# emtiyaz/vmp-for-svae

Measured on AMD Instinct MI355X. Metric: vmp_step_datapoints_per_sec, higher is better.
Workload: dtype f32

## Files before the change

vmp-for-svae_amd/csrc/vmp_mix.hip:

```cpp
#include "vmp_common.h"
#include "vmp_linalg.h"
#include <stdlib.h>
#include <type_traits>

using namespace vmp;

namespace {

constexpr int TR = 64;
constexpr int LS = 68;
constexpr int MAX_NW = 8;
constexpr int MAX_NW1 = 8;
constexpr int max_nw(int KT) { return KT == 1 ? MAX_NW1 : MAX_NW; }
constexpr int MAX_BLOCKS = 1024;

struct PassArgs {
    const float* x;
    const float* r_in;
    const float* u_in;
    const uint8_t* mask;
    const float* pivot;
    const float* pack;
    float* r_out;
    float* u_out;
    float* logr_out;
    double* partials;
    long long N;
    long long rpw;
    long long rpw_b;
    int K;
    int vec_ok;
    int par_reduce;
#ifdef VMP_DEBUG_TS
    long long* dbg_t;
#endif
};
#ifdef VMP_DEBUG_TS
#define PASS_TS(i) do { if (a.dbg_t && (blockIdx.x == 0 || blockIdx.x == 100) && (threadIdx.x & 63) == 0) { a.dbg_t[(blockIdx.x ? 64 : 0) + (threadIdx.x >> 6) * 8 + (i)] = clock64(); \
    if ((i) == 0 && threadIdx.x == 0) a.dbg_t[(blockIdx.x ? 64 : 0) + 7] = wall_clock64();           \
    if ((i) == 5 && threadIdx.x == 64) a.dbg_t[(blockIdx.x ? 64 : 0) + 8 + 7] = wall_clock64(); } } while (0)
#else
#define PASS_TS(i) do { } while (0)
#endif

#define VMP_DPP2(OP, CTRL)                                                   \
    "v_" OP "_f32_dpp %0, %0, %0 " CTRL " row_mask:0xf bank_mask:0xf\n\t"  \
    "v_" OP "_f32_dpp %1, %1, %1 " CTRL " row_mask:0xf bank_mask:0xf\n\t"  \
    "s_nop 0\n\t"
#define VMP_DPP2_FIRST(OP, CTRL)                                             \
    "v_" OP "_f32_dpp %0, %2, %2 " CTRL " row_mask:0xf bank_mask:0xf\n\t"  \
    "v_" OP "_f32_dpp %1, %3, %3 " CTRL " row_mask:0xf bank_mask:0xf\n\t"  \
    "s_nop 0\n\t"
__device__ __forceinline__ v2f row16_max2(v2f v) {
    float a, b;
    asm("s_nop 1\n\t" VMP_DPP2_FIRST("max", "row_ror:8") VMP_DPP2("max", "row_ror:4") VMP_DPP2("max", "row_ror:2")
        VMP_DPP2("max", "row_ror:1")
        : "=&v"(a), "=&v"(b) : "v"(v.x), "v"(v.y));
    return v2f{a, b};
}
__device__ __forceinline__ v2f row16_sum2(v2f v) {
    float a, b;
    asm("s_nop 1\n\t" VMP_DPP2_FIRST("add", "row_ror:8") VMP_DPP2("add", "row_ror:4") VMP_DPP2("add", "row_ror:2")
        VMP_DPP2("add", "row_ror:1")
        : "=&v"(a), "=&v"(b) : "v"(v.x), "v"(v.y));
    return v2f{a, b};
}

#define VMP_DPP4(OP, CTRL)                                                   \
    "v_" OP "_f32_dpp %0, %0, %0 " CTRL " row_mask:0xf bank_mask:0xf\n\t"  \
    "v_" OP "_f32_dpp %1, %1, %1 " CTRL " row_mask:0xf bank_mask:0xf\n\t"  \
    "v_" OP "_f32_dpp %2, %2, %2 " CTRL " row_mask:0xf bank_mask:0xf\n\t"  \
    "v_" OP "_f32_dpp %3, %3, %3 " CTRL " row_mask:0xf bank_mask:0xf\n\t"
#define VMP_DPP4_FIRST(OP, CTRL)                                             \
    "v_" OP "_f32_dpp %0, %4, %4 " CTRL " row_mask:0xf bank_mask:0xf\n\t"  \
    "v_" OP "_f32_dpp %1, %5, %5 " CTRL " row_mask:0xf bank_mask:0xf\n\t"  \
    "v_" OP "_f32_dpp %2, %6, %6 " CTRL " row_mask:0xf bank_mask:0xf\n\t"  \
    "v_" OP "_f32_dpp %3, %7, %7 " CTRL " row_mask:0xf bank_mask:0xf\n\t"
[[maybe_unused]] __device__ __forceinline__ void row16_max4(v2f v0, v2f v1, v2f& o0, v2f& o1) {
    float a, b, c, d;
    asm("s_nop 1\n\t" VMP_DPP4_FIRST("max", "row_ror:8") VMP_DPP4("max", "row_ror:4") VMP_DPP4("max", "row_ror:2")
        VMP_DPP4("max", "row_ror:1")
        : "=&v"(a), "=&v"(b), "=&v"(c), "=&v"(d) : "v"(v0.x), "v"(v0.y), "v"(v1.x), "v"(v1.y));
    o0 = v2f{a, b};
    o1 = v2f{c, d};
}
[[maybe_unused]] __device__ __forceinline__ void row16_sum4(v2f v0, v2f v1, v2f& o0, v2f& o1) {
    float a, b, c, d;
    asm("s_nop 1\n\t" VMP_DPP4_FIRST("add", "row_ror:8") VMP_DPP4("add", "row_ror:4") VMP_DPP4("add", "row_ror:2")
        VMP_DPP4("add", "row_ror:1")
        : "=&v"(a), "=&v"(b), "=&v"(c), "=&v"(d) : "v"(v0.x), "v"(v0.y), "v"(v1.x), "v"(v1.y));
    o0 = v2f{a, b};
    o1 = v2f{c, d};
}

#define VMP_RS4(OP, TAIL)                                                                   \
    "s_nop 1\n\t"                                                                           \
    "v_" OP "_f32_dpp %0, %3, %3 row_ror:8 row_mask:0xf bank_mask:0x3\n\t"                \
    "v_" OP "_f32_dpp %0, %5, %5 row_ror:8 row_mask:0xf bank_mask:0xc\n\t"                \
    "v_" OP "_f32_dpp %1, %4, %4 row_ror:8 row_mask:0xf bank_mask:0x3\n\t"                \
    "v_" OP "_f32_dpp %1, %6, %6 row_ror:8 row_mask:0xf bank_mask:0xc\n\t"                \
    "v_" OP "_f32_dpp %2, %0, %0 row_ror:12 row_mask:0xf bank_mask:0x5\n\t"               \
    "s_nop 0\n\t"                                                                           \
    "v_" OP "_f32_dpp %2, %1, %1 row_ror:4 row_mask:0xf bank_mask:0xa\n\t"                \
    "s_nop 1\n\t"                                                                           \
    "v_" OP "_f32_dpp %2, %2, %2 quad_perm:[2,3,0,1] row_mask:0xf bank_mask:0xf\n\t"      \
    "s_nop 1\n\t"                                                                           \
    "v_" OP "_f32_dpp %2, %2, %2 quad_perm:[1,0,3,2] row_mask:0xf bank_mask:0xf\n\t" TAIL
__device__ __forceinline__ float row16_rs4_max(v2f v0, v2f v1) {
    float a0, a1, b;
    asm(VMP_RS4("max", "s_nop 1\n\t") : "=&v"(a0), "=&v"(a1), "=&v"(b) : "v"(v0.x), "v"(v0.y), "v"(v1.x), "v"(v1.y));
    return b;
}
__device__ __forceinline__ float row16_rs4_sum(v2f v0, v2f v1) {
    float a0, a1, b;
    asm(VMP_RS4("add", "") : "=&v"(a0), "=&v"(a1), "=&v"(b) : "v"(v0.x), "v"(v0.y), "v"(v1.x), "v"(v1.y));
    return b;
}
template <int V>
__device__ __forceinline__ float row16_bcast_bank(float s) {
    return __uint_as_float(__builtin_amdgcn_update_dpp(0u, __float_as_uint(s), 0x150 + 4 * V, 0xf, 0xf, true));
}

#ifndef VMP_PASS_PIPE
#define VMP_PASS_PIPE 4
#endif

constexpr int MOM_TERMS = 3;
#ifndef VMP_MOM_FLUSH
#define VMP_MOM_FLUSH 2
#endif

template <int D, int KT, int FLAV>
__device__ __forceinline__ void pass_epilogue(const PassArgs& a, float* smem, const double (&dacc)[KT][Geo<D>::FT][4],
                                              const double (&dn)[KT][4], int lane, int wave, int nw) {
    using G = Geo<D>;
    constexpr int FT = G::FT;
    constexpr bool SMM = (FLAV == VMP_SMM);
    const int K = a.K;
    {
        __syncthreads();
        PASS_TS(3);
        double* sc = reinterpret_cast<double*>(smem);
        constexpr int SLAB = KT * (FT + 1) * 4 * WAVE;
        if (a.par_reduce) {
            double* mine = sc + wave * SLAB;
#pragma unroll
            for (int kt = 0; kt < KT; ++kt)
#pragma unroll
                for (int c = 0; c < 4; ++c) {
#pragma unroll
                    for (int ft = 0; ft < FT; ++ft) mine[((kt * (FT + 1) + ft) * 4 + c) * WAVE + lane] = dacc[kt][ft][c];
                    mine[((kt * (FT + 1) + FT) * 4 + c) * WAVE + lane] = SMM ? dn[kt][c] : dacc[kt][0][c];
                }
            __syncthreads();
            constexpr int EPT = 2, NWB = max_nw(KT);
            for (int e0 = threadIdx.x; e0 < SLAB; e0 += EPT * blockDim.x) {
                double vals[EPT][NWB];
#pragma unroll
                for (int q = 0; q < EPT; ++q) {
                    const int e = e0 + q * blockDim.x;
#pragma unroll
                    for (int w = 0; w < NWB; ++w) vals[q][w] = (e < SLAB && w < nw) ? sc[w * SLAB + e] : 0.0;
                }
#pragma unroll
                for (int q = 0; q < EPT; ++q) {
                    const int e = e0 + q * blockDim.x;
                    double t2 = vals[q][0];
#pragma unroll
                    for (int w = 1; w < NWB; ++w) t2 += vals[q][w];
                    if (e < SLAB) sc[e] = t2;
                }
            }
            __syncthreads();
        } else {
            for (int w = 0; w < nw; ++w) {
                if (wave == w) {
#pragma unroll
                    for (int kt = 0; kt < KT; ++kt)
#pragma unroll
                        for (int c = 0; c < 4; ++c) {
#pragma unroll
                            for (int ft = 0; ft < FT; ++ft) {
                                const int idx = ((kt * (FT + 1) + ft) * 4 + c) * WAVE + lane;
                                sc[idx] = (w == 0 ? 0.0 : sc[idx]) + dacc[kt][ft][c];
                            }
                            const int idn = ((kt * (FT + 1) + FT) * 4 + c) * WAVE + lane;
                            sc[idn] = (w == 0 ? 0.0 : sc[idn]) + (SMM ? dn[kt][c] : dacc[kt][0][c]);
                        }
                }
                __syncthreads();
            }
        }
        PASS_TS(4);
        constexpr int PX = G::PF + 1;
        double* out = a.partials;
        for (int e = threadIdx.x; e < KT * (FT + 1) * 4 * WAVE; e += blockDim.x) {
            const int l = e & 63, c = (e >> 6) & 3, tf = (e >> 8) % (FT + 1), kt = (e >> 8) / (FT + 1);
            const int k = kt * 16 + (l >> 4) * 4 + c;
            if (k >= K) continue;
            double* row = out + ((long long)k * MAX_BLOCKS + blockIdx.x) * PX;
            if (tf < FT) {
                const int f = tf * 16 + (l & 15);
                if (f < G::F) row[f] = sc[e];
            } else if ((l & 15) == 0) {
                row[G::F] = sc[e];
            }
        }
        if (wave == 0) {
// ... 338 lines not shown
                        av[t] = __builtin_bit_cast(bf16x8, u32x4{As[kt][t][0], As[kt][t][1], As[kt][t][2], As[kt][t][3]});
                        if constexpr (SMM) rv[t] = __builtin_bit_cast(bf16x8, u32x4{Rs[kt][t][0], Rs[kt][t][1], Rs[kt][t][2], Rs[kt][t][3]});
                    }
#pragma unroll
                    for (int ta = 0; ta < MOM_TERMS; ++ta) {
#pragma unroll
                        for (int tb = 0; tb + ta < MOM_TERMS; ++tb) {
#pragma unroll
                            for (int ft = 0; ft < FT; ++ft) {
                                if (ta + tb == 0) acc[kt][ft] = __builtin_amdgcn_mfma_f32_16x16x32_bf16(av[ta], b[ft][tb], acc[kt][ft], 0, 0, 0);
                                else acs[kt][ft] = __builtin_amdgcn_mfma_f32_16x16x32_bf16(av[ta], b[ft][tb], acs[kt][ft], 0, 0, 0);
                            }
                        }
                        if constexpr (SMM) {
                            if (ta == 0) nacc[kt] = __builtin_amdgcn_mfma_f32_16x16x32_bf16(rv[ta], b[0][0], nacc[kt], 0, 0, 0);
                            else nacs[kt] = __builtin_amdgcn_mfma_f32_16x16x32_bf16(rv[ta], b[0][0], nacs[kt], 0, 0, 0);
                        }
                    }
                }
            }
        }

        if constexpr (STATS) {
            if (((row0 - lo) / TR) % VMP_MOM_FLUSH == VMP_MOM_FLUSH - 1 || row0 + TR >= hi) {
#pragma unroll
                for (int kt = 0; kt < KT; ++kt) {
#pragma unroll
                    for (int c = 0; c < 4; ++c) {
                        if constexpr (SMM) dn[kt][c] += (double)nacc[kt][c] + (double)nacs[kt][c];
#pragma unroll
                        for (int ft = 0; ft < FT; ++ft) dacc[kt][ft][c] += (double)acc[kt][ft][c] + (double)acs[kt][ft][c];
                    }
                    nacc[kt] = f32x4{0.f, 0.f, 0.f, 0.f};
                    nacs[kt] = f32x4{0.f, 0.f, 0.f, 0.f};
#pragma unroll
                    for (int ft = 0; ft < FT; ++ft) { acc[kt][ft] = f32x4{0.f, 0.f, 0.f, 0.f}; acs[kt][ft] = f32x4{0.f, 0.f, 0.f, 0.f}; }
                }
            }
        }
        __builtin_amdgcn_wave_barrier();
    }

    PASS_TS(2);
    if constexpr (STATS) pass_epilogue<D, KT, FLAV>(a, smem, dacc, dn, lane, wave, nw);
}


constexpr int AIS = 36;

struct FinArgs {
    const double* partials;
    const double* stats_in;
    int nblk, K, flavour, src, do_post;
    const float *alpha0, *beta0, *m0, *C0, *v0, *kappa;
    const float* pivot;
    float *alpha, *beta, *m, *C, *v, *xbar, *S, *pi, *pack;
    double* pack64;
    double* stats_out;
    double* peer[VMP_EXCH_MAX_RANKS];
    int nranks, rank;
    unsigned long long iter;
    int* status;
#ifdef VMP_DEBUG_TS
    long long* dbg_t;
#endif
};

#ifdef VMP_DEBUG_TS
#define FIN_TS(i) do { if (a.dbg_t && blockIdx.x == 0 && tid == 0) { a.dbg_t[i] = clock64(); if ((i) == 0) a.dbg_t[6] = wall_clock64(); if ((i) == 5) a.dbg_t[7] = wall_clock64(); } } while (0)
#else
#define FIN_TS(i) do { } while (0)
#endif
#ifdef VMP_DEBUG_TS
#define FIN_TSX(i, t) do { if (a.dbg_t && blockIdx.x == 0 && tid == (t)) a.dbg_t[i] = clock64(); } while (0)
#else
#define FIN_TSX(i, t) do { } while (0)
#endif

template <int D>
__device__ void finalize_block(const FinArgs& a, const int k, const int tid, const int nthreads);

template <int D> constexpr int xdl_wave_floats() { return Geo<D>::XROWS * LS + TR * AIS; }

template <int D, int FLAV, bool STATS, int MT = 3>
__device__ __forceinline__ void pass_xdl_body(const PassArgs& a) {
    using G = Geo<D>;
    constexpr int FT = G::FT, KT = 1;
    constexpr bool SMM = (FLAV == VMP_SMM);
    constexpr int DP = (D + 1) / 2;
    extern __shared__ __attribute__((aligned(16))) float smem[];
    const int lane = threadIdx.x & 63, wave = threadIdx.x >> 6, nw = blockDim.x >> 6;
    const int K = a.K;
    PASS_TS(0);
    float* xl = smem + wave * xdl_wave_floats<D>();
    unsigned* ai = reinterpret_cast<unsigned*>(xl + G::XROWS * LS);
    constexpr int ONE = D, ZERO = D + 1;
    const int ppos = (lane & ~15) + 4 * (lane & 3) + ((lane >> 2) & 3);

    const bool vec = a.vec_ok != 0;
    long long lo, hi;
    if (a.rpw_b == a.rpw) {
        lo = ((long long)blockIdx.x * nw + wave) * a.rpw;
        hi = lo + a.rpw;
    } else {
        const int hw = nw >> 1;
        const long long base = (long long)blockIdx.x * hw * (a.rpw + a.rpw_b);
        lo = wave < hw ? base + wave * a.rpw : base + hw * a.rpw + (wave - hw) * a.rpw_b;
        hi = lo + (wave < hw ? a.rpw : a.rpw_b);
    }
    if (hi > a.N) hi = a.N;
    float xr[D];
    {
        const long long n = lo + lane;
#pragma unroll
        for (int j = 0; j < D; ++j) xr[j] = 0.f;
        if (n < hi) load_row<D>(a.x + n * D, xr, vec);
    }
    const int i16 = lane & 15, kk = lane >> 4;
    float pv[D];
    {
        const float* __restrict__ pp = a.pivot ? a.pivot : a.x;
        const bool hasp = a.pivot != nullptr;
#pragma unroll
        for (int j = 0; j < D; ++j) { const float v = pp[j]; pv[j] = hasp ? v : 0.f; }
#pragma unroll
        for (int j = 0; j < D; ++j) pv[j] = __builtin_bit_cast(float, __builtin_amdgcn_readfirstlane(__builtin_bit_cast(int, pv[j])));
    }

    constexpr int NS = D < 4 ? D : 4;
    constexpr int NB = D > 4 ? D - 4 : 0;
    constexpr int QK = 3 * NS + 4 * NB, QS = QK | 1;
    static_assert(16 * QS * 4 <= xdl_wave_floats<D>(), "the operand image must fit the LDS of a one-wave launch");
    u32x4 Bsm[NS], B1[NB > 0 ? NB : 1], B2[NB > 0 ? NB : 1];
    v2f pch;
    float pua, pub;
    {
        const bool on = i16 < K;
        const float* __restrict__ pc = a.pack + (on ? i16 : 0) * G::PACK + D + G::TRI;
        const float c0 = pc[0], c1 = pc[1], c2 = pc[2], c3 = pc[3];
        pch.x = on ? c0 : -INFINITY;
        pch.y = on ? c1 : 0.f;
        pua = on ? c2 : 0.f;
        pub = on ? c3 : 1.f;
    }
    {
        u32x4* img = reinterpret_cast<u32x4*>(smem);
        for (int it = threadIdx.x; it < 16 * D; it += blockDim.x) {
            const int k = it / D, i = it - k * D;
            const bool on = k < K;
            const float* __restrict__ p = a.pack + (on ? k : 0) * G::PACK;
            const int tri = i * (i + 1) / 2;
            float mr[D], wr[D];
#pragma unroll
            for (int j = 0; j < D; ++j) { mr[j] = p[j]; wr[j] = p[D + tri + j]; }
            double bi = 0.0;
#pragma unroll
            for (int j = 0; j < D; ++j)
                if (j <= i) bi -= (double)wr[j] * ((double)mr[j] - (double)pv[j]);
            unsigned tb[3];
            split_bf16<3>(v2f{(float)bi, 0.f}, tb);
            const unsigned bias0 = (tb[0] & 0xffffu) | (tb[1] << 16), bias1 = tb[2] & 0xffffu;
            unsigned th[4] = {0u, 0u, 0u, 0u}, tm[4] = {0u, 0u, 0u, 0u}, tl[4] = {0u, 0u, 0u, 0u};
#pragma unroll
            for (int q = 0; q < DP; ++q) {
                const int j0 = 2 * q, j1 = 2 * q + 1;
                const float wa = j0 <= i ? wr[j0] : 0.f;
                const float wb = (j1 <= i && j1 < D) ? wr[j1 < D ? j1 : 0] : 0.f;
                unsigned t3[3];
                split_bf16<3>(v2f{wa, wb}, t3);
                th[q] = t3[0]; tm[q] = t3[1]; tl[q] = t3[2];
            }
            const u32x4 zero = u32x4{0u, 0u, 0u, 0u};
            const u32x4 bias = on ? u32x4{bias0, bias1, 0u, 0u} : zero;
            if (i < NS) {
                u32x4* o = img + k * QS + 3 * i;
// ... 16 lines not shown
        if constexpr (NB > 0) {
            const int s1 = kk == 1 ? 3 : (kk == 2 ? 1 : 0), s2 = kk == 0 ? 2 : (kk == 1 ? 0 : 1);
#pragma unroll
            for (int ib = 0; ib < NB; ++ib) {
                B1[ib] = q[3 * NS + 4 * ib + s1];
                const u32x4 w2 = q[3 * NS + 4 * ib + s2];
                B2[ib] = kk == 3 ? u32x4{0u, 0u, 0u, 0u} : w2;
            }
        }
        __syncthreads();
    }
    xl[ONE * LS + lane] = 1.0f;
    xl[ZERO * LS + lane] = 0.0f;
    {
        u32x4 ones = u32x4{0x3F803F80u, 0x00003F80u, 0u, 0u}, zeros = u32x4{0u, 0u, 0u, 0u};
        *reinterpret_cast<u32x4*>(ai + lane * AIS + 12) = ones;
        *reinterpret_cast<u32x4*>(ai + lane * AIS + 16) = zeros;
    }
    const int rho = 4 * (i16 & 3) + (i16 >> 2);
    const int offA1 = rho * AIS + (kk == 1 ? 12 : (kk == 3 ? 4 : 0));
    const int offA2 = rho * AIS + (kk == 0 ? 0 : (kk == 1 ? 8 : (kk == 2 ? 4 : 16)));
    const int offA3 = rho * AIS + (kk == 3 ? 12 : 20 + 4 * kk);

    int offA[FT], offB[FT];
#pragma unroll
    for (int ft = 0; ft < FT; ++ft) {
        const int f = ft * 16 + i16;
        int ra = ZERO, rb = ZERO;
        if (f == 0) { ra = ONE; rb = ONE; }
        else if (f <= D) { ra = f - 1; rb = ONE; }
        else if (f < G::F) {
            int p = f - D - 1, d = 0;
            while (p >= D - d) { p -= D - d; ++d; }
            ra = d; rb = d + p;
        }
        offA[ft] = ra * LS + 4 * kk;
        offB[ft] = rb * LS + 4 * kk;
    }

    f32x4 acc[KT][FT], acs[KT][FT];
    double dacc[KT][FT][4];
    double dn[KT][4];
    float nsum = 0.f;
    double dnl = 0.0;
#pragma unroll
    for (int c = 0; c < 4; ++c) dn[0][c] = 0.0;
#pragma unroll
    for (int ft = 0; ft < FT; ++ft) {
        acc[0][ft] = f32x4{0.f, 0.f, 0.f, 0.f};
        acs[0][ft] = f32x4{0.f, 0.f, 0.f, 0.f};
#pragma unroll
        for (int c = 0; c < 4; ++c) dacc[0][ft][c] = 0.0;
    }

#ifdef VMP_DEBUG_TS
    asm volatile("" :: "v"(xr[0]), "v"(pv[0]), "v"(pch.x), "v"(Bsm[0][0]));
    asm volatile("s_waitcnt vmcnt(0)" ::: "memory");
#endif
    PASS_TS(1);
    long long row0 = lo, tbase = 0;
    int trows = TR;
    auto stage = [&](auto whole_c) __attribute__((always_inline)) {
        constexpr bool WHOLE = decltype(whole_c)::value;
        {
            const bool valid = WHOLE || row0 + lane < hi;
            float xs[2 * DP];
#pragma unroll
            for (int j = 0; j < 2 * DP; ++j) xs[j] = (valid && j < D) ? xr[j < D ? j : 0] - pv[j < D ? j : 0] : 0.f;
#pragma unroll
            for (int j = 0; j < D; ++j) xl[j * LS + ppos] = xs[j];
            unsigned th[4] = {0u, 0u, 0u, 0u}, tm[4] = {0u, 0u, 0u, 0u}, tl[4] = {0u, 0u, 0u, 0u};
#pragma unroll
            for (int q = 0; q < DP; ++q) {
                unsigned t3[3];
                split_bf16<3>(v2f{xs[2 * q], xs[2 * q + 1]}, t3);
                th[q] = t3[0]; tm[q] = t3[1]; tl[q] = t3[2];
            }
            *reinterpret_cast<u32x4*>(ai + lane * AIS) = u32x4{th[0], th[1], th[2], th[3]};
            *reinterpret_cast<u32x4*>(ai + lane * AIS + 4) = u32x4{tm[0], tm[1], tm[2], tm[3]};
            *reinterpret_cast<u32x4*>(ai + lane * AIS + 8) = u32x4{tl[0], tl[1], tl[2], tl[3]};
            *reinterpret_cast<u32x4*>(ai + lane * AIS + 20) = u32x4{th[0], th[1], th[0], th[1]};
            *reinterpret_cast<u32x4*>(ai + lane * AIS + 24) = u32x4{tm[0], tm[1], th[0], th[1]};
            *reinterpret_cast<u32x4*>(ai + lane * AIS + 28) = u32x4{tl[0], tl[1], tm[0], tm[1]};
            const long long n2 = row0 + TR + lane;
#pragma unroll
            for (int j = 0; j < D; ++j) xr[j] = 0.f;
            if (n2 < hi) load_row<D>(a.x + n2 * D, xr, vec);
        }
        __builtin_amdgcn_wave_barrier();
        tbase = (row0 + kk) * (WHOLE ? 16 : K) + i16;
    };
    auto body = [&](auto full_c, auto n0_v) __attribute__((always_inline)) {
        constexpr bool FULL = decltype(full_c)::value;
        constexpr bool LINE = !std::is_same<decltype(n0_v), int>::value;
        const int n0 = n0_v;
        unsigned As[3][4], Bs[FT][3][4];
        auto subtile = [&](auto jj_c) __attribute__((always_inline)) {
            constexpr int jj = decltype(jj_c)::value;
            const int n16 = n0 + 16 * jj;
            if (!FULL && n16 >= trows) {
                if constexpr (STATS) {
#pragma unroll
                    for (int t = 0; t < 3; ++t) {
                        As[t][2 * jj] = 0u; As[t][2 * jj + 1] = 0u;
#pragma unroll
                        for (int ft = 0; ft < FT; ++ft) { Bs[ft][t][2 * jj] = 0u; Bs[ft][t][2 * jj + 1] = 0u; }
                    }
                }
                return;
            }
            f32x4 y[D];
            {
                const bf16x8 a3 = __builtin_bit_cast(bf16x8, *reinterpret_cast<const u32x4*>(ai + n16 * AIS + offA3));
#pragma unroll
                for (int i = 0; i < NS; ++i)
                    y[i] = __builtin_amdgcn_mfma_f32_16x16x32_bf16(a3, __builtin_bit_cast(bf16x8, Bsm[i]), f32x4{0.f, 0.f, 0.f, 0.f}, 0, 0, 0);
            }
            if constexpr (NB > 0) {
                const bf16x8 a1 = __builtin_bit_cast(bf16x8, *reinterpret_cast<const u32x4*>(ai + n16 * AIS + offA1));
                const bf16x8 a2 = __builtin_bit_cast(bf16x8, *reinterpret_cast<const u32x4*>(ai + n16 * AIS + offA2));
#pragma unroll
                for (int i = 0; i < NB; ++i)
                    y[4 + i] = __builtin_amdgcn_mfma_f32_16x16x32_bf16(a1, __builtin_bit_cast(bf16x8, B1[i]), f32x4{0.f, 0.f, 0.f, 0.f}, 0, 0, 0);
#pragma unroll
                for (int i = 0; i < NB; ++i)
                    y[4 + i] = __builtin_amdgcn_mfma_f32_16x16x32_bf16(a2, __builtin_bit_cast(bf16x8, B2[i]), y[4 + i], 0, 0, 0);
            }
            f32x4 q4 = y[0] * y[0], q4b = f32x4{0.f, 0.f, 0.f, 0.f};
#pragma unroll
            for (int i = 1; i < D; ++i) {
                if (i & 1) q4b = __builtin_elementwise_fma(y[i], y[i], q4b);
                else q4 = __builtin_elementwise_fma(y[i], y[i], q4);
            }
            q4 += q4b;
            v2f lg[2], uu[2], rr[2], w[2];
#pragma unroll
            for (int h = 0; h < 2; ++h) {
                const v2f qh = v2f{q4[2 * h], q4[2 * h + 1]};
                lg[h] = pk_const_minus_scaled(qh, pch);
                if constexpr (SMM) uu[h] = v2f{pua * __builtin_amdgcn_rcpf(qh.x + pub), pua * __builtin_amdgcn_rcpf(qh.y + pub)};
            }
            if constexpr (LINE && VMP_PASS_PIPE >= 4) {
                static_assert(FULL, "straight-line tiles are whole tiles");
                const float mxs = row16_rs4_max(lg[0], lg[1]);
                lg[0] = v2f{__builtin_amdgcn_exp2f(lg[0].x - row16_bcast_bank<0>(mxs)), __builtin_amdgcn_exp2f(lg[0].y - row16_bcast_bank<1>(mxs))};
                lg[1] = v2f{__builtin_amdgcn_exp2f(lg[1].x - row16_bcast_bank<2>(mxs)), __builtin_amdgcn_exp2f(lg[1].y - row16_bcast_bank<3>(mxs))};
                const float invs = __builtin_amdgcn_rcpf(row16_rs4_sum(lg[0], lg[1]));
                rr[0] = v2f{lg[0].x * row16_bcast_bank<0>(invs), lg[0].y * row16_bcast_bank<1>(invs)};
                rr[1] = v2f{lg[1].x * row16_bcast_bank<2>(invs), lg[1].y * row16_bcast_bank<3>(invs)};
#pragma unroll
                for (int h = 0; h < 2; ++h) w[h] = SMM ? rr[h] * uu[h] : rr[h];
            } else {
                v2f mx[2], ssum[2];
                if constexpr (LINE && VMP_PASS_PIPE >= 3) {
                    row16_max4(lg[0], lg[1], mx[0], mx[1]);
#pragma unroll
                    for (int h = 0; h < 2; ++h) lg[h] = v2f{__builtin_amdgcn_exp2f(lg[h].x - mx[h].x), __builtin_amdgcn_exp2f(lg[h].y - mx[h].y)};
                    row16_sum4(lg[0], lg[1], ssum[0], ssum[1]);
                } else {
#pragma unroll
                    for (int h = 0; h < 2; ++h) {
                        mx[h] = row16_max2(lg[h]);
                        lg[h] = v2f{__builtin_amdgcn_exp2f(lg[h].x - mx[h].x), __builtin_amdgcn_exp2f(lg[h].y - mx[h].y)};
                        ssum[h] = row16_sum2(lg[h]);
                    }
                }
#pragma unroll
                for (int h = 0; h < 2; ++h) {
                    v2f inv = v2f{__builtin_amdgcn_rcpf(ssum[h].x), __builtin_amdgcn_rcpf(ssum[h].y)};
                    if constexpr (!FULL) {
                        const bool va = row0 + n16 + 8 * h + kk < hi, vb = row0 + n16 + 8 * h + 4 + kk < hi;
                        inv = v2f{va ? inv.x : 0.f, vb ? inv.y : 0.f};
                    }
                    rr[h] = lg[h] * inv;
                    w[h] = SMM ? rr[h] * uu[h] : rr[h];
                }
            }
#pragma unroll
            for (int v = 0; v < 4; ++v) {
                const float rv = rr[v >> 1][v & 1];
                if constexpr (FULL) {
                    float* __restrict__ ro = a.r_out + tbase + (long long)(n16 + 4 * v) * 16;
                    __builtin_nontemporal_store(rv, ro);
                    if constexpr (SMM) __builtin_nontemporal_store(uu[v >> 1][v & 1], a.u_out + tbase + (long long)(n16 + 4 * v) * 16);
                    if constexpr (!LINE)
                        if (a.logr_out) a.logr_out[tbase + (long long)(n16 + 4 * v) * 16] = logf(rv);
                } else {
                    const bool sv = (row0 + n16 + 4 * v + kk < hi) && i16 < K;
                    const long long o = tbase + (long long)(n16 + 4 * v) * K;
                    if (sv) {
                        a.r_out[o] = rv;
                        if constexpr (SMM) a.u_out[o] = uu[v >> 1][v & 1];
                        if (a.logr_out) a.logr_out[o] = logf(rv);
                    }
                }
            }
            if constexpr (LINE) {
                if (a.logr_out) {
#pragma unroll
                    for (int v = 0; v < 4; ++v) a.logr_out[tbase + (long long)(n16 + 4 * v) * 16] = logf(rr[v >> 1][v & 1]);
                }
            }
            if constexpr (STATS) {
                unsigned t3[3];
#pragma unroll
                for (int h = 0; h < 2; ++h) {
                    split_bf16<MT>(w[h], t3);
#pragma unroll
                    for (int t = 0; t < 3; ++t) As[t][2 * jj + h] = t3[t];
                }
                if constexpr (SMM) nsum += (rr[0].x + rr[0].y) + (rr[1].x + rr[1].y);
#pragma unroll
                for (int ft = 0; ft < FT; ++ft) {
                    const f32x4 fa = *reinterpret_cast<const f32x4*>(&xl[offA[ft] + n16]);
                    const f32x4 fb = *reinterpret_cast<const f32x4*>(&xl[offB[ft] + n16]);
                    const f32x4 pr = fa * fb;
#pragma unroll
                    for (int h = 0; h < 2; ++h) {
                        split_bf16<MT>(v2f{pr[2 * h], pr[2 * h + 1]}, t3);
#pragma unroll
                        for (int t = 0; t < 3; ++t) Bs[ft][t][2 * jj + h] = t3[t];
                    }
                }
            }
        };
        using std::integral_constant;
        subtile(integral_constant<int, 0>{});
        subtile(integral_constant<int, 1>{});

        if constexpr (STATS) {
            bf16x8 b[FT][3];
#pragma unroll
            for (int ft = 0; ft < FT; ++ft)
#pragma unroll
                for (int t = 0; t < 3; ++t)
                    b[ft][t] = __builtin_bit_cast(bf16x8, u32x4{Bs[ft][t][0], Bs[ft][t][1], Bs[ft][t][2], Bs[ft][t][3]});
            bf16x8 av[3];
#pragma unroll
            for (int t = 0; t < 3; ++t) av[t] = __builtin_bit_cast(bf16x8, u32x4{As[t][0], As[t][1], As[t][2], As[t][3]});
#pragma unroll
            for (int ta = 0; ta < MT; ++ta) {
#pragma unroll
                for (int tb = 0; tb + ta < MT; ++tb) {
#pragma unroll
                    for (int ft = 0; ft < FT; ++ft) {
                        if (ta + tb == 0) acc[0][ft] = __builtin_amdgcn_mfma_f32_16x16x32_bf16(av[ta], b[ft][tb], acc[0][ft], 0, 0, 0);
                        else acs[0][ft] = __builtin_amdgcn_mfma_f32_16x16x32_bf16(av[ta], b[ft][tb], acs[0][ft], 0, 0, 0);
                    }
                }
            }
        }
    };

    auto flush = [&]() __attribute__((always_inline)) {
        if constexpr (STATS) {
            if (((row0 - lo) / TR) % VMP_MOM_FLUSH == VMP_MOM_FLUSH - 1 || row0 + TR >= hi) {
#pragma unroll
                for (int c = 0; c < 4; ++c) {
#pragma unroll
                    for (int ft = 0; ft < FT; ++ft) dacc[0][ft][c] += (double)acc[0][ft][c] + (double)acs[0][ft][c];
                }
                if constexpr (SMM) { dnl += (double)nsum; nsum = 0.f; }
#pragma unroll
                for (int ft = 0; ft < FT; ++ft) { acc[0][ft] = f32x4{0.f, 0.f, 0.f, 0.f}; acs[0][ft] = f32x4{0.f, 0.f, 0.f, 0.f}; }
            }
        }
        __builtin_amdgcn_wave_barrier();
    };

    using std::integral_constant;
    if (K == 16) {
        for (; row0 + TR <= hi; row0 += TR) {
#if VMP_PASS_PIPE == 1
            asm volatile("s_waitcnt vmcnt(0)" ::: "memory");
#endif
            stage(integral_constant<bool, true>{});
            body(integral_constant<bool, true>{}, integral_constant<int, 0>{});
            body(integral_constant<bool, true>{}, integral_constant<int, 32>{});
            flush();
        }
    }
    for (; row0 < hi; row0 += TR) {
        trows = (hi - row0 < TR) ? (int)(hi - row0) : TR;
        stage(integral_constant<bool, false>{});
#pragma unroll 1
        for (int n0 = 0; n0 < trows; n0 += 32) {
            const bool full = (K == 16) && (n0 + 32 <= trows);
            if (full) body(integral_constant<bool, true>{}, n0);
            else body(integral_constant<bool, false>{}, n0);
        }
        flush();
    }

    PASS_TS(2);
    if constexpr (STATS && SMM) {
        double tot = dnl;
        {
            int lo = __double2loint(tot), hi = __double2hiint(tot);
            tot += __hiloint2double(__shfl_xor(hi, 32), __shfl_xor(lo, 32));
            lo = __double2loint(tot); hi = __double2hiint(tot);
            tot += __hiloint2double(__shfl_xor(hi, 16), __shfl_xor(lo, 16));
        }
#pragma unroll
        for (int c = 0; c < 4; ++c) {
            const int src = 4 * kk + c;
            const int lo = __shfl(__double2loint(tot), src), hi = __shfl(__double2hiint(tot), src);
            dn[0][c] = __hiloint2double(hi, lo);
        }
    }
    if constexpr (STATS) pass_epilogue<D, 1, FLAV>(a, smem, dacc, dn, lane, wave, nw);
}

template <int D, int FLAV, bool STATS, int MT = 3>
__global__ __launch_bounds__(MAX_NW1 * WAVE) void pass_xdl_kernel(PassArgs a) {
    pass_xdl_body<D, FLAV, STATS, MT>(a);
}

template <int D>
__device__ void write_pack(float* pack, int k, const double* m, const double* W ,
                           double c, double h, double ua, double ub) {
    using G = Geo<D>;
    float* p = pack + k * G::PACK;
    int idx = D;
    for (int j = 0; j < D; ++j) p[j] = (float)m[j];
    for (int i = 0; i < D; ++i)
        for (int j = 0; j <= i; ++j) p[idx++] = (float)W[i * D + j];
    const double LOG2E = 1.4426950408889634074;
    p[idx++] = (float)(c * LOG2E); p[idx++] = (float)(h * LOG2E); p[idx++] = (float)ua; p[idx++] = (float)ub;
}

__device__ __forceinline__ double fast_rsqrt_d(double x) {
    double y = __builtin_amdgcn_rsq(x);
    y = y * (1.5 - 0.5 * x * y * y);
    y = y * (1.5 - 0.5 * x * y * y);
    return y;
}

template <int D>
__device__ __forceinline__ void wave_chol_inverse(const double* A, int lane, double (&X)[D], double& sumlog, bool& ok) {
    double row[D], rd[D];
#pragma unroll
    for (int e = 0; e < D; ++e)
        row[e] = lane < D ? 0.5 * (A[lane * D + e] + A[e * D + lane]) : (e == lane ? 1.0 : 0.0);
    ok = true;
    double mydiag = 1.0;
#pragma unroll
    for (int j = 0; j < D; ++j) {
        double t = row[j];
#pragma unroll
        for (int p = 0; p < j; ++p) t -= row[p] * readlane_d(row[p], j);
        const double sj = readlane_d(t, j);
        ok = ok && (sj > 0.0);
        rd[j] = fast_rsqrt_d(sj);
        if (lane == j) mydiag = sj;
        row[j] = lane >= j ? t * rd[j] : 0.0;
    }
    double lg = lane < D ? 0.5 * log(mydiag) : 0.0;
    sumlog = 0.0;
#pragma unroll
    for (int j = 0; j < D; ++j) sumlog += readlane_d(lg, j);
#pragma unroll
    for (int i = 0; i < D; ++i) {
        double acc = (i == lane) ? 1.0 : 0.0;
#pragma unroll
        for (int p = 0; p < i; ++p) acc -= readlane_d(row[p], i) * X[p];
        X[i] = acc * rd[i];
    }
}

template <int D>
__device__ void estep_constants(int k, int flavour, double alpha_k, double alpha_sum, double beta_k, double v_k,
                                double logdetP, double kap, double& c, double& h, double& ua, double& ub, double& elp) {
    const double LOG2 = 0.69314718055994530942, PI = 3.14159265358979323846;
    elp = digamma_d(alpha_k) - digamma_d(alpha_sum);
    double sdg = 0.0;
    if (flavour == VMP_GMM) {
        for (int i = 0; i < D; ++i) sdg += digamma_d(0.5 * (v_k + 1.0 + i));
        const double ld = (logdetP > log(1e-20)) ? logdetP : 0.0;
        const double eld = sdg + D * LOG2 + ld;
        c = elp + 0.5 * eld - 0.5 * (D / beta_k);
        h = 0.5; ua = 1.0; ub = 1.0;
    } else {
        for (int i = 0; i < D; ++i) sdg += digamma_d(0.5 * (v_k + i));
        const double eld = sdg + D * LOG2 + logdetP;
        h = 0.5 * (D + kap);
        c = lgamma(0.5 * (D + kap)) - lgamma(0.5 * kap) - 0.5 * D * log(kap * PI) + elp + 0.5 * eld
            - h * (D / beta_k) + log(kap);
        ua = D + kap;
        ub = D / beta_k + kap;
    }
}

constexpr int FIN_THREADS = 1024;
constexpr int FIN_MAX_GROUPS = FIN_THREADS / 64;

__device__ __forceinline__ void st_pack(const FinArgs& a, int idx, double v) {
    a.pack[idx] = (float)v;
    if (a.pack64) a.pack64[idx] = v;
// ... 341 lines not shown
struct PassPlan {
    int form;
    int flavour;
    bool estep, stats, mask;
    int kt_mt;
    int nw, blocks, par_reduce;
    size_t lds;
    long long rpw, rpw_b;
};

#ifndef VMP_SPLIT_GMM
#define VMP_SPLIT_GMM 64
#endif
#ifndef VMP_SPLIT_SMM
#define VMP_SPLIT_SMM 62
#endif
#ifndef VMP_MOM2_ROWS
#define VMP_MOM2_ROWS (1ll << 16)
#endif

PassPlan pass_plan(long long N, int D, int K, int flavour, bool estep, bool stats, bool mask) {
    PassPlan p{};
    if (N < 1 || D < 1 || D > VMP_MAX_D || K < 1 || K > VMP_MAX_K || (flavour != VMP_GMM && flavour != VMP_SMM)) return p;
    if ((!estep && !stats) || (mask && (!estep || stats || flavour != VMP_GMM))) return p;
    p.flavour = flavour; p.estep = estep; p.stats = stats; p.mask = mask;
    const int KTn = (K + 15) / 16;
    const bool xdl = estep && !mask && K <= 16;
    p.form = xdl ? PASS_XDL : PASS_TILED;
    p.kt_mt = xdl ? (stats && N >= VMP_MOM2_ROWS ? 2 : 3) : (KTn <= 2 ? KTn : 4);
    constexpr int tuned_blocks = 256;
    constexpr int tuned_nw = MAX_NW;
    const size_t wreg = (size_t)((D + 2) * LS + (xdl ? TR * AIS : 0)) * sizeof(float);
    int nw = tuned_nw;
    if (nw > max_nw(KTn)) nw = max_nw(KTn);
    if (nw < 1) nw = 1;
    const long long ntiles = (N + TR - 1) / TR;
    if ((long long)nw > ntiles) nw = (int)ntiles;
    long long blocks = (ntiles + nw - 1) / nw;
    if (blocks > tuned_blocks) blocks = tuned_blocks;
    if (blocks > MAX_BLOCKS) blocks = MAX_BLOCKS;
    long long rpw = (N + blocks * nw - 1) / (blocks * nw);
    rpw = (rpw + 7) / 8 * 8;
    if (rpw < TR) rpw = TR;
    blocks = ((N + rpw - 1) / rpw + nw - 1) / nw;
    p.rpw_b = rpw;
    const int split = flavour == VMP_SMM ? VMP_SPLIT_SMM : VMP_SPLIT_GMM;
    if (nw == 8 && split != 50 && rpw >= 2 * TR) {
        long long cap = tuned_blocks < MAX_BLOCKS ? tuned_blocks : MAX_BLOCKS;
        long long pr = ((N + 4 * cap - 1) / (4 * cap) + 7) / 8 * 8;
        if (pr < 2 * TR) pr = 2 * TR;
        const long long ra = (pr * split / 100 + 4) / 8 * 8, rb = pr - ra;
        if (rb >= TR) {
            rpw = ra;
            p.rpw_b = rb;
            blocks = (N + 4 * pr - 1) / (4 * pr);
        }
    }
    p.rpw = rpw;
    p.nw = nw;
    p.blocks = (int)blocks;
    const int FTn = (1 + D + D * (D + 1) / 2 + 15) / 16;
    const size_t scratch = stats ? (size_t)(KTn <= 2 ? KTn : 4) * (FTn + 1) * 4 * WAVE * sizeof(double) : 0;
    p.lds = wreg * nw;
    p.par_reduce = 0;
    if (scratch * nw <= 64 * 1024) {
        p.par_reduce = 1;
        if (scratch * nw > p.lds) p.lds = scratch * nw;
    } else if (scratch > p.lds) {
        p.lds = scratch;
    }
    return p;
}

int partial_rows(long long N, int D, int K, int flavour) {
    return pass_plan(N, D, K, flavour == VMP_SMM ? VMP_SMM : VMP_GMM, false, true, false).blocks;
}

template <int D, int KT, int FL, bool E, bool S, bool M>
int launch_tiled(const PassArgs& a, const PassPlan& p, hipStream_t s) {
    hipLaunchKernelGGL((pass_kernel<D, KT, FL, E, S, M>), dim3(p.blocks), dim3(p.nw * WAVE), p.lds, s, a);
    return check_launch("pass_kernel");
}

template <int D, int FL, bool S, int MT>
int launch_xdl(const PassArgs& a, const PassPlan& p, hipStream_t s) {
    if (p.lds > 64 * 1024) {
        if (const int rc = set_dyn_lds(reinterpret_cast<const void*>(pass_xdl_kernel<D, FL, S, MT>), p.lds, "pass_xdl_kernel")) return rc;
    }
    hipLaunchKernelGGL((pass_xdl_kernel<D, FL, S, MT>), dim3(p.blocks), dim3(p.nw * WAVE), p.lds, s, a);
    return check_launch("pass_xdl_kernel");
}

template <int D, int KT, int FL>
int launch_tiled_form(const PassArgs& a, const PassPlan& p, hipStream_t s) {
    if (!p.estep) return launch_tiled<D, KT, FL, false, true, false>(a, p, s);
    if (p.stats) return launch_tiled<D, KT, FL, true, true, false>(a, p, s);
    if constexpr (FL == VMP_GMM) {
        if (p.mask) return launch_tiled<D, KT, FL, true, false, true>(a, p, s);
    }
    return launch_tiled<D, KT, FL, true, false, false>(a, p, s);
}

template <int D, int FL>
int launch_pass(const PassArgs& a, const PassPlan& p, hipStream_t s) {
    if (p.form == PASS_XDL) {
        if (!p.stats) return launch_xdl<D, FL, false, 3>(a, p, s);
        return p.kt_mt == 2 ? launch_xdl<D, FL, true, 2>(a, p, s) : launch_xdl<D, FL, true, 3>(a, p, s);
    }
    switch (p.kt_mt) {
        case 1: return launch_tiled_form<D, 1, FL>(a, p, s);
        case 2: return launch_tiled_form<D, 2, FL>(a, p, s);
        default: return launch_tiled_form<D, 4, FL>(a, p, s);
    }
}

int check_dims(int64_t N, int D, int K) {
    if (N <= 0) { set_error("N must be positive (got %lld)", (long long)N); return VMP_E_BADARG; }
    if (D < 1 || D > VMP_MAX_D) { set_error("D=%d outside compiled range 1..%d", D, VMP_MAX_D); return VMP_E_DIM; }
    if (K < 1 || K > VMP_MAX_K) { set_error("K=%d outside compiled range 1..%d", K, VMP_MAX_K); return VMP_E_DIM; }
    return 0;
}

#ifdef VMP_DEBUG_TS
static long long* g_dbg_pass = nullptr;
static long long* g_dbg_t = nullptr;
#endif
int run_pass(PassArgs a, int D, int flavour, bool estep, bool stats, hipStream_t s) {
    const PassPlan p = pass_plan(a.N, D, a.K, flavour, estep, stats, a.mask != nullptr);
    if (p.form == PASS_NONE) {
        set_error("mixture pass: no kernel for flavour %d, estep %d, stats %d, mask %d", flavour, (int)estep, (int)stats, (int)(a.mask != nullptr));
        return VMP_E_BADARG;
    }
    a.rpw = p.rpw;
    a.rpw_b = p.rpw_b;
    a.par_reduce = p.par_reduce;
#ifdef VMP_DEBUG_TS
    a.dbg_t = g_dbg_pass;
#endif

    int rc = -1;
    VMP_SWITCH_DIM(D, DD, rc = flavour == VMP_SMM ? launch_pass<DD, VMP_SMM>(a, p, s) : launch_pass<DD, VMP_GMM>(a, p, s));
    return rc;
}

int run_finalize(FinArgs f, int D, hipStream_t s) {
    int rc = -1;
#ifdef VMP_DEBUG_TS
    f.dbg_t = g_dbg_t;
#endif

    VMP_SWITCH_DIM(D, DD, {
        hipLaunchKernelGGL((finalize_kernel<DD>), dim3(f.K), dim3(FIN_THREADS), 0, s, f);
        rc = check_launch("finalize_kernel");
    });
    return rc;
}

struct AccArgs { const float* x; const double* pack; float* r; float* u; float* logr; long long N; int K; };
template <int D, bool SMM>
__global__ __launch_bounds__(256) void estep_f64_kernel(AccArgs a) {
    using G = Geo<D>;
    extern __shared__ double spk[];
    for (int e = threadIdx.x; e < a.K * G::PACK; e += blockDim.x) spk[e] = a.pack[e];
    __syncthreads();
    const double LN2 = 0.69314718055994530942;
    for (long long n = (long long)blockIdx.x * blockDim.x + threadIdx.x; n < a.N; n += (long long)gridDim.x * blockDim.x) {
        double xd[D];
#pragma unroll
        for (int j = 0; j < D; ++j) xd[j] = (double)a.x[n * D + j];
        auto quad = [&](int k) {
            const double* __restrict__ p = spk + k * G::PACK;
            double q = 0.0;
#pragma unroll
// ... 389 lines not shown
```

Baseline: 24.09 billion.

## Add K=16 overlap kernel that handles tail rows with a shifted whole tile

Adds a specialized XDL pass kernel for K==16 in which each wave's partial last tile is replaced by a full straight-line tile shifted back to end at the wave's row limit. Rows already processed are masked out of the statistics through a threshold. The generic per-32-row slow path for tails is avoided, and K becomes a compile-time constant. It also removes the unused VMP_PASS_PIPE variants and the row16_max4/sum4 helpers. The host picks the overlap kernel when K is 16 and every wave has at least one full tile, at the cost of recomputing some rows.

```diff
diff --git a/vmp-for-svae_amd/csrc/vmp_mix.hip b/vmp-for-svae_amd/csrc/vmp_mix.hip
--- a/vmp-for-svae_amd/csrc/vmp_mix.hip
+++ b/vmp-for-svae_amd/csrc/vmp_mix.hip
@@ -66,33 +66,6 @@
     return v2f{a, b};
 }
 
-#define VMP_DPP4(OP, CTRL)                                                   \
-    "v_" OP "_f32_dpp %0, %0, %0 " CTRL " row_mask:0xf bank_mask:0xf\n\t"  \
-    "v_" OP "_f32_dpp %1, %1, %1 " CTRL " row_mask:0xf bank_mask:0xf\n\t"  \
-    "v_" OP "_f32_dpp %2, %2, %2 " CTRL " row_mask:0xf bank_mask:0xf\n\t"  \
-    "v_" OP "_f32_dpp %3, %3, %3 " CTRL " row_mask:0xf bank_mask:0xf\n\t"
-#define VMP_DPP4_FIRST(OP, CTRL)                                             \
-    "v_" OP "_f32_dpp %0, %4, %4 " CTRL " row_mask:0xf bank_mask:0xf\n\t"  \
-    "v_" OP "_f32_dpp %1, %5, %5 " CTRL " row_mask:0xf bank_mask:0xf\n\t"  \
-    "v_" OP "_f32_dpp %2, %6, %6 " CTRL " row_mask:0xf bank_mask:0xf\n\t"  \
-    "v_" OP "_f32_dpp %3, %7, %7 " CTRL " row_mask:0xf bank_mask:0xf\n\t"
-[[maybe_unused]] __device__ __forceinline__ void row16_max4(v2f v0, v2f v1, v2f& o0, v2f& o1) {
-    float a, b, c, d;
-    asm("s_nop 1\n\t" VMP_DPP4_FIRST("max", "row_ror:8") VMP_DPP4("max", "row_ror:4") VMP_DPP4("max", "row_ror:2")
-        VMP_DPP4("max", "row_ror:1")
-        : "=&v"(a), "=&v"(b), "=&v"(c), "=&v"(d) : "v"(v0.x), "v"(v0.y), "v"(v1.x), "v"(v1.y));
-    o0 = v2f{a, b};
-    o1 = v2f{c, d};
-}
-[[maybe_unused]] __device__ __forceinline__ void row16_sum4(v2f v0, v2f v1, v2f& o0, v2f& o1) {
-    float a, b, c, d;
-    asm("s_nop 1\n\t" VMP_DPP4_FIRST("add", "row_ror:8") VMP_DPP4("add", "row_ror:4") VMP_DPP4("add", "row_ror:2")
-        VMP_DPP4("add", "row_ror:1")
-        : "=&v"(a), "=&v"(b), "=&v"(c), "=&v"(d) : "v"(v0.x), "v"(v0.y), "v"(v1.x), "v"(v1.y));
-    o0 = v2f{a, b};
-    o1 = v2f{c, d};
-}
-
 #define VMP_RS4(OP, TAIL)                                                                   \
     "s_nop 1\n\t"                                                                           \
     "v_" OP "_f32_dpp %0, %3, %3 row_ror:8 row_mask:0xf bank_mask:0x3\n\t"                \
@@ -120,10 +93,6 @@
 __device__ __forceinline__ float row16_bcast_bank(float s) {
     return __uint_as_float(__builtin_amdgcn_update_dpp(0u, __float_as_uint(s), 0x150 + 4 * V, 0xf, 0xf, true));
 }
-
-#ifndef VMP_PASS_PIPE
-#define VMP_PASS_PIPE 4
-#endif
 
 constexpr int MOM_TERMS = 3;
 #ifndef VMP_MOM_FLUSH
@@ -628,7 +597,7 @@
 
 template <int D> constexpr int xdl_wave_floats() { return Geo<D>::XROWS * LS + TR * AIS; }
 
-template <int D, int FLAV, bool STATS, int MT = 3>
+template <int D, int FLAV, bool STATS, int MT = 3, bool GEN = true>
 __device__ __forceinline__ void pass_xdl_body(const PassArgs& a) {
     using G = Geo<D>;
     constexpr int FT = G::FT, KT = 1;
@@ -636,7 +605,7 @@
     constexpr int DP = (D + 1) / 2;
     extern __shared__ __attribute__((aligned(16))) float smem[];
     const int lane = threadIdx.x & 63, wave = threadIdx.x >> 6, nw = blockDim.x >> 6;
-    const int K = a.K;
+    const int K = GEN ? a.K : 16;
     PASS_TS(0);
     float* xl = smem + wave * xdl_wave_floats<D>();
     unsigned* ai = reinterpret_cast<unsigned*>(xl + G::XROWS * LS);
@@ -819,7 +788,9 @@
             *reinterpret_cast<u32x4*>(ai + lane * AIS + 20) = u32x4{th[0], th[1], th[0], th[1]};
             *reinterpret_cast<u32x4*>(ai + lane * AIS + 24) = u32x4{tm[0], tm[1], th[0], th[1]};
             *reinterpret_cast<u32x4*>(ai + lane * AIS + 28) = u32x4{tl[0], tl[1], tm[0], tm[1]};
-            const long long n2 = row0 + TR + lane;
+            long long nb = row0 + TR;
+            if (!GEN && WHOLE && nb < hi && nb > hi - TR) nb = hi - TR;
+            const long long n2 = nb + lane;
 #pragma unroll
             for (int j = 0; j < D; ++j) xr[j] = 0.f;
             if (n2 < hi) load_row<D>(a.x + n2 * D, xr, vec);
@@ -827,9 +798,12 @@
         __builtin_amdgcn_wave_barrier();
         tbase = (row0 + kk) * (WHOLE ? 16 : K) + i16;
     };
-    auto body = [&](auto full_c, auto n0_v) __attribute__((always_inline)) {
+    int othr = 0;
+    auto body = [&](auto full_c, auto n0_v, auto ovl_c) __attribute__((always_inline)) {
         constexpr bool FULL = decltype(full_c)::value;
         constexpr bool LINE = !std::is_same<decltype(n0_v), int>::value;
+        constexpr bool OVL = decltype(ovl_c)::value;
+        static_assert(!OVL || LINE, "only a straight-line tile overlaps");
         const int n0 = n0_v;
         unsigned As[3][4], Bs[FT][3][4];
         auto subtile = [&](auto jj_c) __attribute__((always_inline)) {
@@ -877,7 +851,7 @@
                 lg[h] = pk_const_minus_scaled(qh, pch);
                 if constexpr (SMM) uu[h] = v2f{pua * __builtin_amdgcn_rcpf(qh.x + pub), pua * __builtin_amdgcn_rcpf(qh.y + pub)};
             }
-            if constexpr (LINE && VMP_PASS_PIPE >= 4) {
+            if constexpr (LINE) {
                 static_assert(FULL, "straight-line tiles are whole tiles");
                 const float mxs = row16_rs4_max(lg[0], lg[1]);
                 lg[0] = v2f{__builtin_amdgcn_exp2f(lg[0].x - row16_bcast_bank<0>(mxs)), __builtin_amdgcn_exp2f(lg[0].y - row16_bcast_bank<1>(mxs))};
@@ -889,18 +863,11 @@
                 for (int h = 0; h < 2; ++h) w[h] = SMM ? rr[h] * uu[h] : rr[h];
             } else {
                 v2f mx[2], ssum[2];
-                if constexpr (LINE && VMP_PASS_PIPE >= 3) {
-                    row16_max4(lg[0], lg[1], mx[0], mx[1]);
-#pragma unroll
-                    for (int h = 0; h < 2; ++h) lg[h] = v2f{__builtin_amdgcn_exp2f(lg[h].x - mx[h].x), __builtin_amdgcn_exp2f(lg[h].y - mx[h].y)};
-                    row16_sum4(lg[0], lg[1], ssum[0], ssum[1]);
-                } else {
-#pragma unroll
-                    for (int h = 0; h < 2; ++h) {
-                        mx[h] = row16_max2(lg[h]);
-                        lg[h] = v2f{__builtin_amdgcn_exp2f(lg[h].x - mx[h].x), __builtin_amdgcn_exp2f(lg[h].y - mx[h].y)};
-                        ssum[h] = row16_sum2(lg[h]);
-                    }
+#pragma unroll
+                for (int h = 0; h < 2; ++h) {
+                    mx[h] = row16_max2(lg[h]);
+                    lg[h] = v2f{__builtin_amdgcn_exp2f(lg[h].x - mx[h].x), __builtin_amdgcn_exp2f(lg[h].y - mx[h].y)};
+                    ssum[h] = row16_sum2(lg[h]);
                 }
 #pragma unroll
                 for (int h = 0; h < 2; ++h) {
@@ -939,6 +906,14 @@
                 }
             }
             if constexpr (STATS) {
+                if constexpr (OVL) {
+#pragma unroll
+                    for (int h = 0; h < 2; ++h) {
+                        const bool ka = n16 + 8 * h >= othr, kb = n16 + 8 * h + 4 >= othr;
+                        w[h] = v2f{ka ? w[h].x : 0.f, kb ? w[h].y : 0.f};
+                        if constexpr (SMM) rr[h] = v2f{ka ? rr[h].x : 0.f, kb ? rr[h].y : 0.f};
+                    }
+                }
                 unsigned t3[3];
 #pragma unroll
                 for (int h = 0; h < 2; ++h) {
@@ -1006,27 +981,46 @@
     };
 
     using std::integral_constant;
-    if (K == 16) {
+    using T_ = integral_constant<bool, true>;
+    using F_ = integral_constant<bool, false>;
+    if constexpr (!GEN) {
         for (; row0 + TR <= hi; row0 += TR) {
-#if VMP_PASS_PIPE == 1
-            asm volatile("s_waitcnt vmcnt(0)" ::: "memory");
-#endif
-            stage(integral_constant<bool, true>{});
-            body(integral_constant<bool, true>{}, integral_constant<int, 0>{});
-            body(integral_constant<bool, true>{}, integral_constant<int, 32>{});
+            stage(T_{});
+            body(T_{}, integral_constant<int, 0>{}, F_{});
+            body(T_{}, integral_constant<int, 32>{}, F_{});
             flush();
         }
-    }
-    for (; row0 < hi; row0 += TR) {
-        trows = (hi - row0 < TR) ? (int)(hi - row0) : TR;
-        stage(integral_constant<bool, false>{});
+        PASS_TS(6);
+        if (row0 < hi && hi - lo >= TR) {
+            const int done = TR - (int)(hi - row0);
+            row0 = hi - TR;
+            othr = done - kk;
+            stage(T_{});
+            if (done < 32) body(T_{}, integral_constant<int, 0>{}, T_{});
+            body(T_{}, integral_constant<int, 32>{}, T_{});
+            flush();
+        }
+    } else {
+        if (K == 16) {
+            for (; row0 + TR <= hi; row0 += TR) {
+                stage(T_{});
+                body(T_{}, integral_constant<int, 0>{}, F_{});
+                body(T_{}, integral_constant<int, 32>{}, F_{});
+                flush();
+            }
+        }
+        PASS_TS(6);
+        for (; row0 < hi; row0 += TR) {
+            trows = (hi - row0 < TR) ? (int)(hi - row0) : TR;
+            stage(F_{});
 #pragma unroll 1
-        for (int n0 = 0; n0 < trows; n0 += 32) {
-            const bool full = (K == 16) && (n0 + 32 <= trows);
-            if (full) body(integral_constant<bool, true>{}, n0);
-            else body(integral_constant<bool, false>{}, n0);
-        }
-        flush();
+            for (int n0 = 0; n0 < trows; n0 += 32) {
+                const bool full = (K == 16) && (n0 + 32 <= trows);
+                if (full) body(T_{}, n0, F_{});
+                else body(F_{}, n0, F_{});
+            }
+            flush();
+        }
     }
 
     PASS_TS(2);
@@ -1050,7 +1044,11 @@
 
 template <int D, int FLAV, bool STATS, int MT = 3>
 __global__ __launch_bounds__(MAX_NW1 * WAVE) void pass_xdl_kernel(PassArgs a) {
-    pass_xdl_body<D, FLAV, STATS, MT>(a);
+    pass_xdl_body<D, FLAV, STATS, MT, true>(a);
+}
+template <int D, int FLAV, bool STATS, int MT = 3>
+__global__ __launch_bounds__(MAX_NW1 * WAVE) void pass_xdl_overlap_kernel(PassArgs a) {
+    pass_xdl_body<D, FLAV, STATS, MT, false>(a);
 }
 
 template <int D>
@@ -1558,13 +1556,29 @@
     return check_launch("pass_kernel");
 }
 
+template <int D, int FL, bool S, int MT, bool GEN>
+int launch_xdl_form(const PassArgs& a, const PassPlan& p, hipStream_t s) {
+    void (*const kern)(PassArgs) = GEN ? pass_xdl_kernel<D, FL, S, MT> : pass_xdl_overlap_kernel<D, FL, S, MT>;
+    if (p.lds > 64 * 1024) {
+        if (const int rc = set_dyn_lds(reinterpret_cast<const void*>(kern), p.lds, "pass_xdl_kernel")) return rc;
+    }
+    hipLaunchKernelGGL(kern, dim3(p.blocks), dim3(p.nw * WAVE), p.lds, s, a);
+    return check_launch("pass_xdl_kernel");
+}
+
+long long last_wave_rows(const PassPlan& p, long long N) {
+    if (p.rpw_b == p.rpw) return N - (N - 1) / p.rpw * p.rpw;
+    const long long hw = p.nw / 2, per = hw * (p.rpw + p.rpw_b);
+    long long rem = N - (N - 1) / per * per;
+    if (rem <= hw * p.rpw) return rem - (rem - 1) / p.rpw * p.rpw;
+    rem -= hw * p.rpw;
+    return rem - (rem - 1) / p.rpw_b * p.rpw_b;
+}
+
 template <int D, int FL, bool S, int MT>
 int launch_xdl(const PassArgs& a, const PassPlan& p, hipStream_t s) {
-    if (p.lds > 64 * 1024) {
-        if (const int rc = set_dyn_lds(reinterpret_cast<const void*>(pass_xdl_kernel<D, FL, S, MT>), p.lds, "pass_xdl_kernel")) return rc;
-    }
-    hipLaunchKernelGGL((pass_xdl_kernel<D, FL, S, MT>), dim3(p.blocks), dim3(p.nw * WAVE), p.lds, s, a);
-    return check_launch("pass_xdl_kernel");
+    const bool line = a.K == 16 && last_wave_rows(p, a.N) >= TR;
+    return line ? launch_xdl_form<D, FL, S, MT, false>(a, p, s) : launch_xdl_form<D, FL, S, MT, true>(a, p, s);
 }
 
 template <int D, int KT, int FL>
```

New measurement: 24.36 billion (median of 6 runs). 1.01x the previous value.
